# dusk-network/schnorr

Measured on NVIDIA B200. Metric: verifies_per_s, higher is better.
Workload: dtype u32

## Files before the change

schnorr_b200/csrc/constants_gen.cuh:

```cuda
#pragma once
#include <cstdint>
namespace sb200 {
#define SB200_FQ_MOD_INIT {0x00000001u, 0xffffffffu, 0xfffe5bfeu, 0x53bda402u, 0x09a1d805u, 0x3339d808u, 0x299d7d48u, 0x73eda753u}
#define SB200_FR_MOD_INIT {0xd6f72cb7u, 0xd0970e5eu, 0xccc81082u, 0xa6682093u, 0x01343b00u, 0x06673b01u, 0x6533afa9u, 0x0e7db4eau}
#define SB200_8R_INIT {0xb7b965b8u, 0x84b872f6u, 0x66408416u, 0x3341049eu, 0x09a1d805u, 0x3339d808u, 0x299d7d48u, 0x73eda753u}
#define SB200_FQ_ONE_INIT {0xfffffffeu, 0x00000001u, 0x00034802u, 0x5884b7fau, 0xecbc4ff5u, 0x998c4fefu, 0xacc5056fu, 0x1824b159u}
#define SB200_FQ_R2_INIT {0xf3f29c6du, 0xc999e990u, 0x87925c23u, 0x2b6cedcbu, 0x7254398fu, 0x05d31496u, 0x9f59ff11u, 0x0748d9d9u}
#define SB200_FR_R2_INIT {0x95e57731u, 0x67719aa4u, 0x9ce3fc26u, 0x51b0cef0u, 0xc026e9a5u, 0x69dab7fau, 0x8d127688u, 0x04f6547bu}
#define SB200_FR_NINV 0xef788ef9u
#define SB200_FQ_NINV 0xffffffffu
#define SB200_ED_D_INIT {0xb974f6b0u, 0x2a522455u, 0x0d9acab3u, 0xfc6cc9efu, 0xc27628d1u, 0x7a08fb94u, 0xfe0e262eu, 0x57f8f6a8u}
#define SB200_ED_2D_INIT {0x72e9ed5fu, 0x54a448acu, 0x1b373967u, 0xa51befdbu, 0x7b4a799eu, 0xc0d81f21u, 0xd27ecf14u, 0x3c0445feu}
#define SB200_G_U_INIT {0x547c71aau, 0xc8cd898cu, 0xb3564650u, 0x1e77bad0u, 0x49031ebeu, 0x0b5183a6u, 0xa3031a2cu, 0x4f54a483u}
#define SB200_G_V_INIT {0xffffffd9u, 0x00000026u, 0x003ffc27u, 0x3e1c038bu, 0x88581730u, 0x323016c6u, 0xa901ea00u, 0x56cb8254u}
#define SB200_GP_U_INIT {0x71c3e812u, 0x51d37e72u, 0x2074aaa8u, 0xf3ad4539u, 0xc0cfbca7u, 0x21bb2537u, 0x8bf29c9cu, 0x0bb82922u}
#define SB200_GP_V_INIT {0x0c68cf00u, 0x36fba2bfu, 0xd2b7f2adu, 0xcd442b52u, 0xf9f895d4u, 0xbe025c79u, 0x466dbd00u, 0x61e43e3fu}
#define SB200_FQ_ROOT_OF_UNITY_INIT {0x5f0e466au, 0xb9b58d8cu, 0x1819d7ecu, 0x5b1b4c80u, 0x52a31e64u, 0x0af53ae3u, 0x19e9b27bu, 0x5bf3addau}
#define SB200_FQ_SQRT_EXP_INIT {0x7fffffffu, 0x7fff2dffu, 0xa9ded201u, 0x04d0ec02u, 0x199cec04u, 0x94cebea4u, 0x39f6d3a9u, 0x00000000u}
#define SB200_FQ_SQRT_EXP_BITS 222
#define SB200_FQ_ISQRT_EXP_INIT {0x80000000u, 0x8000d1ffu, 0x561f89fdu, 0x4eecb800u, 0xf004ec01u, 0x9e6b1963u, 0xefa6a99eu, 0x73eda752u}
#define SB200_FQ_ISQRT_EXP_BITS 255
#define SB200_FQ_DLOG_W_INIT { \
  {0xfffffffeu, 0x00000001u, 0x00034802u, 0x5884b7fau, 0xecbc4ff5u, 0x998c4fefu, 0xacc5056fu, 0x1824b159u}, \
  {0x88202b65u, 0x1acf64e4u, 0x819f004fu, 0x5b18b637u, 0x3107fdf5u, 0xee649cabu, 0xce9012a0u, 0x27a8543du}, \
  {0x2c42eff8u, 0x6ecf4995u, 0x4d5dfa57u, 0x6ec1fa83u, 0x5656b15cu, 0x3ff5cf38u, 0x229e031bu, 0x54b80267u}, \
  {0x45c09c96u, 0x5fb40c77u, 0x8b8b1b1bu, 0xfff59b78u, 0x6b7eed47u, 0x023ba68bu, 0x76f3e130u, 0x4e17f66fu}, \
  {0xaa89cfb1u, 0xf3b05674u, 0x6006b9feu, 0x072f0140u, 0x25667a26u, 0xce9a0dbfu, 0x2d598374u, 0x4d2ce405u}, \
  {0x0b0a1289u, 0x25c2a002u, 0x7d082188u, 0x971c717fu, 0xd81ac5d8u, 0x4739dccau, 0xeee341c1u, 0x4f607ba9u}, \
  {0x3eb2a8ddu, 0x111f9842u, 0x6f38b840u, 0x1f772784u, 0x8e3ca13cu, 0xb28758a3u, 0xed9a48f0u, 0x5974f9f7u}, \
  {0xdcbeed53u, 0x0ddd2e46u, 0x33dbdd55u, 0xdf977d7fu, 0xc1470bbau, 0xdda3b36au, 0xb67a22b2u, 0x4818fbf6u}, \
  {0x00000003u, 0xfffffffdu, 0xfffb13fcu, 0xfb38ec08u, 0x1ce5880fu, 0x99ad8818u, 0x7cd877d8u, 0x5bc8f5f9u}, \
  {0x77dfd49cu, 0xe5309b1au, 0x7e5f5bafu, 0xf8a4edcbu, 0xd899da0fu, 0x44d53b5cu, 0x5b0d6aa7u, 0x4c455315u}, \
  {0xd3bd1009u, 0x9130b669u, 0xb2a061a7u, 0xe4fba97fu, 0xb34b26a8u, 0xf34408cfu, 0x06ff7a2cu, 0x1f35a4ecu}, \
  {0xba3f636bu, 0xa04bf387u, 0x747340e3u, 0x53c8088au, 0x9e22eabdu, 0x30fe317cu, 0xb2a99c18u, 0x25d5b0e3u}, \
  {0x55763050u, 0x0c4fa98au, 0x9ff7a200u, 0x4c8ea2c2u, 0xe43b5ddfu, 0x649fca48u, 0xfc43f9d3u, 0x26c0c34du}, \
  {0xf4f5ed78u, 0xda3d5ffcu, 0x82f63a76u, 0xbca13283u, 0x3187122cu, 0xebfffb3du, 0x3aba3b86u, 0x248d2ba9u}, \
  {0xc14d5724u, 0xeee067bcu, 0x90c5a3beu, 0x34467c7eu, 0x7b6536c9u, 0x80b27f64u, 0x3c033457u, 0x1a78ad5bu}, \
  {0x234112aeu, 0xf222d1b8u, 0xcc227ea9u, 0x74262683u, 0x485acc4au, 0x5596249du, 0x73235a95u, 0x2bd4ab5cu}, \
}
#define SB200_FQ_DLOG_P_INIT { \
  {0xfffffffeu, 0x00000001u, 0x00034802u, 0x5884b7fau, 0xecbc4ff5u, 0x998c4fefu, 0xacc5056fu, 0x1824b159u}, \
  {0xdcf3219au, 0x4256481au, 0x96b6cad3u, 0x45f37b7fu, 0x5f7a3b27u, 0xf9c3f1d7u, 0x658afd43u, 0x2d2fc049u}, \
  {0xb510e57eu, 0x1e4739c8u, 0x184b8322u, 0xcc6032ecu, 0x984f6527u, 0x67262f63u, 0x87e5e5d4u, 0x5f5b959au}, \
  {0x55ba3b5bu, 0x2c18ffe6u, 0xa301cb77u, 0x9f7c110du, 0x8987dc47u, 0xdc5921a2u, 0xb7e50ed6u, 0x2624052cu}, \
  {0x70de2c18u, 0x0491bcebu, 0x87989fc9u, 0xfe592990u, 0xb064bd3cu, 0x687fc87au, 0xfbd5ad87u, 0x184857c8u}, \
  {0x15d8086bu, 0x7da1ec25u, 0x0f895256u, 0xebefe178u, 0x6da44d28u, 0x7ccb4492u, 0x1418b341u, 0x0d341d07u}, \
  {0xa39260bdu, 0x371f6f57u, 0xb2adfd57u, 0x03233f13u, 0xe86e03e8u, 0xda6056f1u, 0x89616101u, 0x64e6ed21u}, \
  {0x5d68adabu, 0xc6213a40u, 0xf0bc64ebu, 0x717d6528u, 0x5a40ec6fu, 0x455a4aefu, 0x8c10c91du, 0x4b3801e3u}, \
  {0x54eb1d75u, 0x79675917u, 0xd07fc645u, 0x1d44be7du, 0x47873890u, 0x1fddcce9u, 0xd4a502f9u, 0x1c9bd17eu}, \
  {0xf41614dbu, 0x91d36fb2u, 0x2d5ee4f0u, 0xf0ca4660u, 0x97a3d0e0u, 0x358061cfu, 0x398358a9u, 0x1f710187u}, \
  {0x0e975eb0u, 0x573de590u, 0xfde6df69u, 0x45876f88u, 0x6fefa181u, 0x8ec11e78u, 0x47e325c6u, 0x3b82fc93u}, \
  {0x44c7342bu, 0x7d6cc6f9u, 0x9d3b75c2u, 0x5f804e66u, 0xfb977827u, 0xc787ac1bu, 0x242122d5u, 0x27cb0565u}, \
  {0x76ab126fu, 0xeda7545bu, 0x02493555u, 0xe69a0018u, 0xd36a1a77u, 0xbf43e82fu, 0x740a2463u, 0x66d7e2d2u}, \
  {0x287def7au, 0x25e3cfcbu, 0xf520ad2eu, 0x33e06f94u, 0xb53a8083u, 0x441ae296u, 0x9ac05dc5u, 0x4e335a86u}, \
  {0xd961433fu, 0x8b753cbdu, 0xb5ef3ca5u, 0x5510c621u, 0xdbe2dc3du, 0x1aed0940u, 0xbf547affu, 0x41202b7au}, \
  {0xd9f2b2e9u, 0x9ad76de6u, 0x69662643u, 0x767ed606u, 0x510ae26bu, 0x6f9e9b13u, 0x6b4afe61u, 0x6aea05a3u}, \
  {0xfffffffeu, 0x00000001u, 0x00034802u, 0x5884b7fau, 0xecbc4ff5u, 0x998c4fefu, 0xacc5056fu, 0x1824b159u}, \
  {0x7b483997u, 0x25909fe2u, 0x3f40368fu, 0xe6c3383bu, 0xdfbf158fu, 0xe7a72791u, 0x90ca2226u, 0x2bccc288u}, \
  {0x61b4a6dfu, 0x3bbb6d5fu, 0xb34eca42u, 0x029e0c54u, 0x3ffd89d1u, 0x1d4e3056u, 0xd07ec38bu, 0x6b3cb83cu}, \
  {0x2fe00938u, 0x6c0ecbb6u, 0xb0e2f081u, 0x464ce985u, 0x63e9f431u, 0x281f3d36u, 0x3c63c33du, 0x151b140du}, \
  {0x27c562bbu, 0xf6d82dbfu, 0x2b57637fu, 0x4ddc7290u, 0x06eab0a9u, 0xc17c34cdu, 0x2b59d621u, 0x068dfbaeu}, \
  {0x7f332db5u, 0x550dd9d7u, 0x50500ad0u, 0x7fc2c5eau, 0xa154e5f1u, 0x68b6c255u, 0x5175c276u, 0x6a14b04au}, \
  {0x3d579818u, 0xeac47c6du, 0xbd12a148u, 0x04cdb7a3u, 0x99cc35bau, 0xc74160d9u, 0x7ded3fd6u, 0x31552226u}, \
  {0x45feca49u, 0x07022427u, 0xe4b9af79u, 0x67ae65c8u, 0x33cd2d6bu, 0xd2aa9542u, 0x766209d0u, 0x4b7f6e39u}, \
  {0xae32dcdeu, 0xbd56d684u, 0x1409bd44u, 0x2db07b79u, 0x76a3e44eu, 0xf6fc95fcu, 0x24ed7b31u, 0x5adc0a48u}, \
  {0x9b8ac597u, 0x18faac24u, 0xad6a2e5eu, 0x03c5535eu, 0x1aeaa4c7u, 0x9516a609u, 0x0e93a59du, 0x4cf2c66fu}, \
  {0xb053e34bu, 0x22b855f1u, 0xa6a58337u, 0x99d367e2u, 0x6a6fed50u, 0x1a1b8fc9u, 0xaf1243eeu, 0x02be6719u}, \
  {0x56a1b05au, 0x4c899974u, 0x52a00333u, 0x92077279u, 0x3fb3e264u, 0x5b69a565u, 0xfd04f965u, 0x22894c17u}, \
  {0x76d4f9a2u, 0xaab13750u, 0x27b6e4cdu, 0x6e15f748u, 0xaad66ed8u, 0x5934218eu, 0x8b7fc61eu, 0x2d8fee11u}, \
  {0x22ba096cu, 0xda0e363bu, 0xe108034au, 0x73e94e78u, 0x03175cb2u, 0x16662707u, 0xdc289c5cu, 0x0935b070u}, \
  {0xba91d935u, 0x8710449fu, 0x10ba6380u, 0x74297a3cu, 0x3ed48ec8u, 0x1944fd71u, 0x230d1a6fu, 0x253baa10u}, \
  {0x45af1cb2u, 0x9912839cu, 0x0eff7d88u, 0x94ce8b8fu, 0x45d2192fu, 0x3d960b14u, 0xa970bf7eu, 0x0ab3e280u}, \
  {0xfffffffeu, 0x00000001u, 0x00034802u, 0x5884b7fau, 0xecbc4ff5u, 0x998c4fefu, 0xacc5056fu, 0x1824b159u}, \
  {0x990adacau, 0xad970bf0u, 0x35d536acu, 0xfcc75b77u, 0x776dcbaeu, 0x8dce37c6u, 0x0b26861du, 0x39f39d66u}, \
  {0x3f3f7413u, 0x62a17c8au, 0xbb17edbau, 0xf60c53c0u, 0x0c4e2817u, 0x4a9ea2d0u, 0xf7c560f3u, 0x13b632eeu}, \
  {0xbf8d2010u, 0xaa23c71fu, 0x1803ba5bu, 0x82408b4cu, 0xb0e69d63u, 0xe205f14cu, 0xc89b398eu, 0x35817d11u}, \
  {0xf6421a00u, 0x52c40fb8u, 0x5ec95569u, 0xbf33428eu, 0x0f71a346u, 0x5ecc78ddu, 0x9336bf44u, 0x5bb66cdbu}, \
  {0xd7a69137u, 0x9d39ae58u, 0xc8b94ac3u, 0x31aa9c79u, 0x01df0186u, 0x165f9fecu, 0xd00f8128u, 0x37fcf0ecu}, \
  {0x8830c83bu, 0xc5ad52beu, 0x3e94bc59u, 0x335c2573u, 0xf405e823u, 0x3e0d24a9u, 0xc983967du, 0x340c1cd8u}, \
  {0x5015e046u, 0xe0e15508u, 0x07f09bf5u, 0x89a013dbu, 0x756f0918u, 0x6a372ae3u, 0xa1a1661eu, 0x3f38e644u}, \
  {0xe3c30b08u, 0x9aa2ba63u, 0xd67b21bcu, 0xc3a07402u, 0x29af6349u, 0x64a4e583u, 0xf6ae051cu, 0x64bffb89u}, \
  {0x97e8c141u, 0x5c0656e3u, 0xde2270f4u, 0x9d2b3e00u, 0x0724a33au, 0x639a4ba0u, 0x8342d321u, 0x081ccecbu}, \
  {0x5eb65c76u, 0x2eb03e83u, 0x7c9d4f12u, 0x01c1e452u, 0x48471ba3u, 0x53c1e14fu, 0x46fa1afdu, 0x57191969u}, \
  {0x40374953u, 0x2176d8ceu, 0x348adbefu, 0xd5f2b8e9u, 0x0192e4aeu, 0x009ddad0u, 0x139e2bedu, 0x062b6996u}, \
  {0xc54c7224u, 0xa473141bu, 0x677c3a87u, 0xe5cc4b84u, 0xd657177cu, 0xc43f284bu, 0x13ede9e1u, 0x68f92b69u}, \
  {0x61e3b145u, 0xace2b2b2u, 0xb79bac80u, 0xe6ee1368u, 0x39d8c96bu, 0xcbc23989u, 0x7bdc8336u, 0x1679bcf7u}, \
  {0x19606f59u, 0x5e54cc69u, 0x72106cf8u, 0x9cc664a2u, 0xa8f39d52u, 0x7ac51b8au, 0xda01f7b5u, 0x6f6436c3u}, \
  {0xc1ce4a7au, 0xf0f3c50bu, 0x1b61b4a3u, 0xd3b7deadu, 0x360f0e9fu, 0x91827a03u, 0x6c77c17au, 0x6ac60dd2u}, \
  {0xfffffffeu, 0x00000001u, 0x00034802u, 0x5884b7fau, 0xecbc4ff5u, 0x998c4fefu, 0xacc5056fu, 0x1824b159u}, \
  {0xb64957f6u, 0x68ee7cb8u, 0x0a2b8bafu, 0x8eeda81eu, 0x256c4becu, 0xd749ce3du, 0x2ae8d689u, 0x48230b86u}, \
// ... 211 lines not shown
```

schnorr_b200/csrc/fq.cuh:

```cuda
#pragma once
#include <cstdint>

#include "constants_gen.cuh"

#if defined(__CUDACC__)
#define SB_HD __host__ __device__ __forceinline__
#define SB_D __device__ __forceinline__
#else
#define SB_HD inline
#define SB_D inline
#endif

namespace sb200 {

#ifndef SB_Q1_SHORTCUT
#define SB_Q1_SHORTCUT 0
#endif

struct fq {
  uint32_t v[8];
};

#if !defined(__CUDA_ARCH__)
namespace emu {
// ... 56 lines not shown
      "madc.lo.cc.u32 %6, %9, %13, %6;\n\t"
      "madc.hi.cc.u32 %7, %9, %13, %7;\n\t"
      "addc.u32 %8, %8, 0;"
      : "+r"(x[0]), "+r"(x[1]), "+r"(x[2]), "+r"(x[3]), "+r"(x[4]), "+r"(x[5]), "+r"(x[6]), "+r"(x[7]), "+r"(ytop)
      : "r"(a), "r"(b0), "r"(b2), "r"(b4), "r"(b6));
#else
  SB_COUNT(wide, 4);
  uint32_t c = emu::add_at(x, 8, 0, (uint64_t)a * b0, 0);
  c += emu::add_at(x, 8, 2, (uint64_t)a * b2, 0);
  c += emu::add_at(x, 8, 4, (uint64_t)a * b4, 0);
  c += emu::add_at(x, 8, 6, (uint64_t)a * b6, 0);
  ytop += c;
#endif
}

SB_HD void blk_mac_odd(uint32_t* y, uint32_t a, uint32_t b1, uint32_t b3, uint32_t b5, uint32_t b7) {
#if defined(__CUDA_ARCH__)
  asm("mad.lo.cc.u32 %0, %8, %9, %0;\n\t"
      "madc.hi.cc.u32 %1, %8, %9, %1;\n\t"
      "madc.lo.cc.u32 %2, %8, %10, %2;\n\t"
      "madc.hi.cc.u32 %3, %8, %10, %3;\n\t"
      "madc.lo.cc.u32 %4, %8, %11, %4;\n\t"
      "madc.hi.cc.u32 %5, %8, %11, %5;\n\t"
      "madc.lo.cc.u32 %6, %8, %12, %6;\n\t"
      "madc.hi.u32 %7, %8, %12, %7;"
      : "+r"(y[0]), "+r"(y[1]), "+r"(y[2]), "+r"(y[3]), "+r"(y[4]), "+r"(y[5]), "+r"(y[6]), "+r"(y[7])
      : "r"(a), "r"(b1), "r"(b3), "r"(b5), "r"(b7));
#else
  SB_COUNT(wide, 4);
  uint32_t c = emu::add_at(y, 8, 0, (uint64_t)a * b1, 0);
  c += emu::add_at(y, 8, 2, (uint64_t)a * b3, 0);
  c += emu::add_at(y, 8, 4, (uint64_t)a * b5, 0);
  c += emu::add_at(y, 8, 6, (uint64_t)a * b7, 0);
  (void)c;
#endif
}

SB_HD void blk_red_even_q(uint32_t* x, uint32_t& ytop, uint32_t m, uint32_t q2, uint32_t q4, uint32_t q6) {
#if defined(__CUDA_ARCH__)
  asm("mad.lo.cc.u32 %0, %7, %8, %0;\n\t"
      "madc.hi.cc.u32 %1, %7, %8, %1;\n\t"
      "madc.lo.cc.u32 %2, %7, %9, %2;\n\t"
      "madc.hi.cc.u32 %3, %7, %9, %3;\n\t"
      "madc.lo.cc.u32 %4, %7, %10, %4;\n\t"
      "madc.hi.cc.u32 %5, %7, %10, %5;\n\t"
      "addc.u32 %6, %6, 0;"
      : "+r"(x[2]), "+r"(x[3]), "+r"(x[4]), "+r"(x[5]), "+r"(x[6]), "+r"(x[7]), "+r"(ytop)
      : "r"(m), "r"(q2), "r"(q4), "r"(q6));
#else
  SB_COUNT(wide, 3);
  uint32_t c = emu::add_at(x, 8, 2, (uint64_t)m * q2, 0);
  c += emu::add_at(x, 8, 4, (uint64_t)m * q4, 0);
  c += emu::add_at(x, 8, 6, (uint64_t)m * q6, 0);
  ytop += c;
#endif
}

SB_HD void blk_red_odd_q(uint32_t* y, uint32_t m, uint32_t t0, uint32_t q3, uint32_t q5, uint32_t q7) {
#if defined(__CUDA_ARCH__)
  asm("{\n\t.reg .u32 h;\n\t"
      "min.u32 h, %8, 1;\n\t"
      "sub.u32 h, %8, h;\n\t"
      "add.cc.u32 %0, %0, %9;\n\t"
      "addc.cc.u32 %1, %1, h;\n\t"
      "madc.lo.cc.u32 %2, %8, %10, %2;\n\t"
      "madc.hi.cc.u32 %3, %8, %10, %3;\n\t"
      "madc.lo.cc.u32 %4, %8, %11, %4;\n\t"
      "madc.hi.cc.u32 %5, %8, %11, %5;\n\t"
      "madc.lo.cc.u32 %6, %8, %12, %6;\n\t"
      "madc.hi.u32 %7, %8, %12, %7;\n\t}"
      : "+r"(y[0]), "+r"(y[1]), "+r"(y[2]), "+r"(y[3]), "+r"(y[4]), "+r"(y[5]), "+r"(y[6]), "+r"(y[7])
      : "r"(m), "r"(t0), "r"(q3), "r"(q5), "r"(q7));
#else
  SB_COUNT(wide, 3);
  uint32_t hi1 = m - (m != 0 ? 1u : 0u);
  uint32_t c = emu::add_at(y, 8, 0, ((uint64_t)hi1 << 32) | t0, 0);
  c += emu::add_at(y, 8, 2, (uint64_t)m * q3, 0);
  c += emu::add_at(y, 8, 4, (uint64_t)m * q5, 0);
  c += emu::add_at(y, 8, 6, (uint64_t)m * q7, 0);
  (void)c;
#endif
}

SB_HD void blk_mac1c(uint32_t* acc, uint32_t a, uint32_t b0) {
#if defined(__CUDA_ARCH__)
  asm("mad.lo.cc.u32 %0, %3, %4, %0;\n\t"
      "madc.hi.cc.u32 %1, %3, %4, %1;\n\t"
      "addc.u32 %2, %2, 0;"
      : "+r"(acc[0]), "+r"(acc[1]), "+r"(acc[2])
      : "r"(a), "r"(b0));
#else
  SB_COUNT(wide, 1);
  acc[2] += emu::add_at(acc, 2, 0, (uint64_t)a * b0, 0);
#endif
}
SB_HD void blk_mac2c(uint32_t* acc, uint32_t a, uint32_t b0, uint32_t b1) {
#if defined(__CUDA_ARCH__)
  asm("mad.lo.cc.u32 %0, %5, %6, %0;\n\t"
      "madc.hi.cc.u32 %1, %5, %6, %1;\n\t"
      "madc.lo.cc.u32 %2, %5, %7, %2;\n\t"
      "madc.hi.cc.u32 %3, %5, %7, %3;\n\t"
      "addc.u32 %4, %4, 0;"
      : "+r"(acc[0]), "+r"(acc[1]), "+r"(acc[2]), "+r"(acc[3]), "+r"(acc[4])
      : "r"(a), "r"(b0), "r"(b1));
#else
  SB_COUNT(wide, 2);
  uint32_t c = emu::add_at(acc, 4, 0, (uint64_t)a * b0, 0);
  c += emu::add_at(acc, 4, 2, (uint64_t)a * b1, 0);
  acc[4] += c;
#endif
}
SB_HD void blk_mac3c(uint32_t* acc, uint32_t a, uint32_t b0, uint32_t b1, uint32_t b2) {
#if defined(__CUDA_ARCH__)
  asm("mad.lo.cc.u32 %0, %7, %8, %0;\n\t"
      "madc.hi.cc.u32 %1, %7, %8, %1;\n\t"
      "madc.lo.cc.u32 %2, %7, %9, %2;\n\t"
      "madc.hi.cc.u32 %3, %7, %9, %3;\n\t"
      "madc.lo.cc.u32 %4, %7, %10, %4;\n\t"
      "madc.hi.cc.u32 %5, %7, %10, %5;\n\t"
      "addc.u32 %6, %6, 0;"
      : "+r"(acc[0]), "+r"(acc[1]), "+r"(acc[2]), "+r"(acc[3]), "+r"(acc[4]), "+r"(acc[5]), "+r"(acc[6])
      : "r"(a), "r"(b0), "r"(b1), "r"(b2));
#else
  SB_COUNT(wide, 3);
  uint32_t c = emu::add_at(acc, 6, 0, (uint64_t)a * b0, 0);
  c += emu::add_at(acc, 6, 2, (uint64_t)a * b1, 0);
  c += emu::add_at(acc, 6, 4, (uint64_t)a * b2, 0);
  acc[6] += c;
#endif
}
SB_HD void blk_mac4c(uint32_t* acc, uint32_t a, uint32_t b0, uint32_t b1, uint32_t b2, uint32_t b3) {
  blk_mac_even(acc, acc[8], a, b0, b1, b2, b3);
}

SB_HD void blk_sqr_diag(uint32_t* t, const uint32_t* a) {
#if defined(__CUDA_ARCH__)
  asm("mad.lo.cc.u32 %0, %16, %16, %0;\n\t"
      "madc.hi.cc.u32 %1, %16, %16, %1;\n\t"
      "madc.lo.cc.u32 %2, %17, %17, %2;\n\t"
      "madc.hi.cc.u32 %3, %17, %17, %3;\n\t"
      "madc.lo.cc.u32 %4, %18, %18, %4;\n\t"
      "madc.hi.cc.u32 %5, %18, %18, %5;\n\t"
      "madc.lo.cc.u32 %6, %19, %19, %6;\n\t"
      "madc.hi.cc.u32 %7, %19, %19, %7;\n\t"
      "madc.lo.cc.u32 %8, %20, %20, %8;\n\t"
      "madc.hi.cc.u32 %9, %20, %20, %9;\n\t"
      "madc.lo.cc.u32 %10, %21, %21, %10;\n\t"
      "madc.hi.cc.u32 %11, %21, %21, %11;\n\t"
      "madc.lo.cc.u32 %12, %22, %22, %12;\n\t"
      "madc.hi.cc.u32 %13, %22, %22, %13;\n\t"
      "madc.lo.cc.u32 %14, %23, %23, %14;\n\t"
      "madc.hi.u32 %15, %23, %23, %15;"
      : "+r"(t[0]), "+r"(t[1]), "+r"(t[2]), "+r"(t[3]), "+r"(t[4]), "+r"(t[5]), "+r"(t[6]), "+r"(t[7]), "+r"(t[8]),
        "+r"(t[9]), "+r"(t[10]), "+r"(t[11]), "+r"(t[12]), "+r"(t[13]), "+r"(t[14]), "+r"(t[15])
      : "r"(a[0]), "r"(a[1]), "r"(a[2]), "r"(a[3]), "r"(a[4]), "r"(a[5]), "r"(a[6]), "r"(a[7]));
#else
  SB_COUNT(wide, 8);
  uint32_t c = 0;
  for (int i = 0; i < 8; i++) c += emu::add_at(t, 16, 2 * i, (uint64_t)a[i] * a[i], 0);
  (void)c;
#endif
}

SB_HD void merge_eo16(uint32_t* r, const uint32_t* e, const uint32_t* o) {
#if defined(__CUDA_ARCH__)
  r[0] = e[0];
  asm("add.cc.u32 %0, %15, %30;\n\t"
      "addc.cc.u32 %1, %16, %31;\n\t"
      "addc.cc.u32 %2, %17, %32;\n\t"
      "addc.cc.u32 %3, %18, %33;\n\t"
      "addc.cc.u32 %4, %19, %34;\n\t"
      "addc.cc.u32 %5, %20, %35;\n\t"
      "addc.cc.u32 %6, %21, %36;\n\t"
      "addc.cc.u32 %7, %22, %37;\n\t"
      "addc.cc.u32 %8, %23, %38;\n\t"
      "addc.cc.u32 %9, %24, %39;\n\t"
      "addc.cc.u32 %10, %25, %40;\n\t"
      "addc.cc.u32 %11, %26, %41;\n\t"
      "addc.cc.u32 %12, %27, %42;\n\t"
      "addc.cc.u32 %13, %28, %43;\n\t"
      "addc.u32 %14, %29, %44;"
      : "=r"(r[1]), "=r"(r[2]), "=r"(r[3]), "=r"(r[4]), "=r"(r[5]), "=r"(r[6]), "=r"(r[7]), "=r"(r[8]), "=r"(r[9]),
        "=r"(r[10]), "=r"(r[11]), "=r"(r[12]), "=r"(r[13]), "=r"(r[14]), "=r"(r[15])
      : "r"(e[1]), "r"(e[2]), "r"(e[3]), "r"(e[4]), "r"(e[5]), "r"(e[6]), "r"(e[7]), "r"(e[8]), "r"(e[9]), "r"(e[10]),
        "r"(e[11]), "r"(e[12]), "r"(e[13]), "r"(e[14]), "r"(e[15]), "r"(o[0]), "r"(o[1]), "r"(o[2]), "r"(o[3]), "r"(o[4]),
        "r"(o[5]), "r"(o[6]), "r"(o[7]), "r"(o[8]), "r"(o[9]), "r"(o[10]), "r"(o[11]), "r"(o[12]), "r"(o[13]), "r"(o[14]));
#else
  r[0] = e[0];
  uint64_t c = 0;
  for (int i = 1; i < 16; i++) {
    c += (uint64_t)e[i] + o[i - 1];
    r[i] = (uint32_t)c;
    c >>= 32;
  }
#endif
}

SB_HD uint32_t blk_fold_red_odd(uint32_t& x0, uint32_t xf, uint32_t tprev, uint32_t* y, uint32_t q1, uint32_t q3,
                                uint32_t q5, uint32_t q7) {
  uint32_t m;
#if defined(__CUDA_ARCH__)
  asm("{\n\t.reg .u32 t, h;\n\t"
      "add.cc.u32 t, %11, 0xffffffff;\n\t"
      "addc.cc.u32 %0, %0, %10;\n\t"
      "xor.b32 %9, %0, %12;\n\t"
      "add.u32 %9, %9, 1;\n\t"
      "min.u32 h, %9, 1;\n\t"
      "sub.u32 h, %9, h;\n\t"
      "addc.cc.u32 %1, %1, %0;\n\t"
      "addc.cc.u32 %2, %2, h;\n\t"
      "madc.lo.cc.u32 %3, %9, %13, %3;\n\t"
      "madc.hi.cc.u32 %4, %9, %13, %4;\n\t"
      "madc.lo.cc.u32 %5, %9, %14, %5;\n\t"
      "madc.hi.cc.u32 %6, %9, %14, %6;\n\t"
      "madc.lo.cc.u32 %7, %9, %15, %7;\n\t"
      "madc.hi.u32 %8, %9, %15, %8;\n\t}"
      : "+r"(x0), "+r"(y[0]), "+r"(y[1]), "+r"(y[2]), "+r"(y[3]), "+r"(y[4]), "+r"(y[5]), "+r"(y[6]), "+r"(y[7]), "=&r"(m)
      : "r"(xf), "r"(tprev), "r"(q1), "r"(q3), "r"(q5), "r"(q7));
#else
  SB_COUNT(wide, 4);
  uint64_t t = (uint64_t)x0 + xf + (tprev != 0 ? 1u : 0u);
  x0 = (uint32_t)t;
  uint32_t c = (uint32_t)(t >> 32);
  m = 0u - x0;
  SB_COUNT(wide, -1);
  (void)q1;
  c = emu::add_at(y, 8, 0, ((uint64_t)(m - (m != 0 ? 1u : 0u)) << 32) | x0, c);
  c += emu::add_at(y, 8, 2, (uint64_t)m * q3, 0);
  c += emu::add_at(y, 8, 4, (uint64_t)m * q5, 0);
  c += emu::add_at(y, 8, 6, (uint64_t)m * q7, 0);
  (void)c;
#endif
  return m;
}

SB_HD uint32_t add8(uint32_t* r, const uint32_t* a, const uint32_t* b) {
  uint32_t c;
#if defined(__CUDA_ARCH__)
  asm("add.cc.u32 %0, %9, %17;\n\t"
      "addc.cc.u32 %1, %10, %18;\n\t"
      "addc.cc.u32 %2, %11, %19;\n\t"
      "addc.cc.u32 %3, %12, %20;\n\t"
      "addc.cc.u32 %4, %13, %21;\n\t"
// ... 204 lines not shown
  mul_wide16(T, a.v, b.v);
  return mont_reduce16(T);
#endif
  uint32_t X[8], Y[8], xf = 0, tprev = 0;
#pragma unroll
  for (int i = 0; i < 8; i++) X[i] = Y[i] = 0;
  const uint32_t q1 = SB_FQ_MOD(1), q2 = SB_FQ_MOD(2), q3 = SB_FQ_MOD(3), q4 = SB_FQ_MOD(4), q5 = SB_FQ_MOD(5),
                 q6 = SB_FQ_MOD(6), q7 = SB_FQ_MOD(7);
#pragma unroll
  for (int i = 0; i < 8; i++) {
    uint32_t ai = a.v[i];
    blk_fold_mac_odd(X[0], xf, tprev, Y, ai, b.v[1], b.v[3], b.v[5], b.v[7]);
    blk_mac_even(X, Y[7], ai, b.v[0], b.v[2], b.v[4], b.v[6]);
    tprev = X[0];
#if defined(__CUDA_ARCH__) && SB_FQ_MOD_IMM
    uint32_t m;
    asm("xor.b32 %0, %1, %2;\n\tadd.u32 %0, %0, 1;" : "=r"(m) : "r"(tprev), "r"(q1));
#else
    uint32_t m = (tprev ^ q1) + 1u;
#endif
    blk_red_even_q(X, Y[7], m, q2, q4, q6);
#if SB_Q1_SHORTCUT
    blk_red_odd_q(Y, m, tprev, q3, q5, q7);
#else
    blk_mac_odd(Y, m, q1, q3, q5, q7);
#endif
    xf = X[1];
    uint32_t nx[8], ny[8];
#pragma unroll
    for (int k = 0; k < 8; k++) nx[k] = Y[k];
#pragma unroll
    for (int k = 0; k < 6; k++) ny[k] = X[k + 2];
    ny[6] = 0;
    ny[7] = 0;
#pragma unroll
    for (int k = 0; k < 8; k++) {
      X[k] = nx[k];
      Y[k] = ny[k];
    }
  }
  fq r;
  uint32_t s[8] = {xf, Y[0], Y[1], Y[2], Y[3], Y[4], Y[5], Y[6]};
  add8c(r.v, X, s, tprev);
  cond_sub_p<FqP>(r.v);
  return r;
}

SB_HD fq mont_reduce16(const uint32_t* t) {
  uint32_t X[8], Y[8], xf = 0, tprev = 0;
#pragma unroll
  for (int i = 0; i < 8; i++) {
    X[i] = t[i];
    Y[i] = 0;
  }
  const uint32_t q1 = SB_FQ_MOD(1), q2 = SB_FQ_MOD(2), q3 = SB_FQ_MOD(3), q4 = SB_FQ_MOD(4), q5 = SB_FQ_MOD(5),
                 q6 = SB_FQ_MOD(6), q7 = SB_FQ_MOD(7);
#pragma unroll
  for (int i = 0; i < 8; i++) {
    uint32_t m = blk_fold_red_odd(X[0], xf, tprev, Y, q1, q3, q5, q7);
    tprev = X[0];
    blk_red_even_q(X, Y[7], m, q2, q4, q6);
    xf = X[1];
    uint32_t nx[8], ny[8];
#pragma unroll
    for (int k = 0; k < 8; k++) nx[k] = Y[k];
#pragma unroll
    for (int k = 0; k < 6; k++) ny[k] = X[k + 2];
    ny[6] = 0;
    ny[7] = 0;
#pragma unroll
    for (int k = 0; k < 8; k++) {
      X[k] = nx[k];
      Y[k] = ny[k];
    }
  }
  fq v, r;
  uint32_t s[8] = {xf, Y[0], Y[1], Y[2], Y[3], Y[4], Y[5], Y[6]};
  add8c(v.v, X, s, tprev);
  add8(r.v, v.v, t + 8);
  cond_sub_p<FqP>(r.v);
  return r;
}

SB_HD fq fq_sqr_inl(const fq& x) {
  SB_COUNT(fq_sqr, 1);
  const uint32_t* a = x.v;
  uint32_t E[16], O[16];
#pragma unroll
  for (int i = 0; i < 16; i++) E[i] = O[i] = 0;
  blk_mac4c(O + 0, a[0], a[1], a[3], a[5], a[7]);
  blk_mac3c(E + 2, a[0], a[2], a[4], a[6]);
  blk_mac3c(O + 2, a[1], a[2], a[4], a[6]);
  blk_mac3c(E + 4, a[1], a[3], a[5], a[7]);
  blk_mac3c(O + 4, a[2], a[3], a[5], a[7]);
  blk_mac2c(E + 6, a[2], a[4], a[6]);
  blk_mac2c(O + 6, a[3], a[4], a[6]);
  blk_mac2c(E + 8, a[3], a[5], a[7]);
  blk_mac2c(O + 8, a[4], a[5], a[7]);
  blk_mac1c(E + 10, a[4], a[6]);
  blk_mac1c(O + 10, a[5], a[6]);
  blk_mac1c(E + 12, a[5], a[7]);
  blk_mac1c(O + 12, a[6], a[7]);
  uint32_t S[16], T[16];
  merge_eo16(S, E, O);
  T[0] = S[0] << 1;
#pragma unroll
  for (int i = 1; i < 16; i++) T[i] = (S[i] << 1) | (S[i - 1] >> 31);
  blk_sqr_diag(T, a);
  return mont_reduce16(T);
}

SB_HD void mul_wide16(uint32_t* T, const uint32_t* a, const uint32_t* b) {
  uint32_t E[18], O[18];
#pragma unroll
  for (int i = 0; i < 18; i++) E[i] = O[i] = 0;
#pragma unroll
  for (int i = 0; i < 8; i++) {
    if ((i & 1) == 0) {
      blk_mac4c(E + i, a[i], b[0], b[2], b[4], b[6]);
      blk_mac4c(O + i, a[i], b[1], b[3], b[5], b[7]);
    } else {
      blk_mac4c(O + i - 1, a[i], b[0], b[2], b[4], b[6]);
      blk_mac4c(E + i + 1, a[i], b[1], b[3], b[5], b[7]);
    }
  }
  merge_eo16(T, E, O);
}

SB_HD void acc17(uint32_t* S, const uint32_t* T) {
#if defined(__CUDA_ARCH__)
  asm("add.cc.u32 %0, %0, %17;\n\t"
      "addc.cc.u32 %1, %1, %18;\n\t"
      "addc.cc.u32 %2, %2, %19;\n\t"
      "addc.cc.u32 %3, %3, %20;\n\t"
      "addc.cc.u32 %4, %4, %21;\n\t"
      "addc.cc.u32 %5, %5, %22;\n\t"
      "addc.cc.u32 %6, %6, %23;\n\t"
      "addc.cc.u32 %7, %7, %24;\n\t"
      "addc.cc.u32 %8, %8, %25;\n\t"
      "addc.cc.u32 %9, %9, %26;\n\t"
      "addc.cc.u32 %10, %10, %27;\n\t"
      "addc.cc.u32 %11, %11, %28;\n\t"
      "addc.cc.u32 %12, %12, %29;\n\t"
      "addc.cc.u32 %13, %13, %30;\n\t"
      "addc.cc.u32 %14, %14, %31;\n\t"
      "addc.cc.u32 %15, %15, %32;\n\t"
      "addc.u32 %16, %16, 0;"
      : "+r"(S[0]), "+r"(S[1]), "+r"(S[2]), "+r"(S[3]), "+r"(S[4]), "+r"(S[5]), "+r"(S[6]), "+r"(S[7]), "+r"(S[8]),
        "+r"(S[9]), "+r"(S[10]), "+r"(S[11]), "+r"(S[12]), "+r"(S[13]), "+r"(S[14]), "+r"(S[15]), "+r"(S[16])
      : "r"(T[0]), "r"(T[1]), "r"(T[2]), "r"(T[3]), "r"(T[4]), "r"(T[5]), "r"(T[6]), "r"(T[7]), "r"(T[8]), "r"(T[9]),
        "r"(T[10]), "r"(T[11]), "r"(T[12]), "r"(T[13]), "r"(T[14]), "r"(T[15]));
#else
  uint64_t c = 0;
  for (int i = 0; i < 16; i++) {
    c += (uint64_t)S[i] + T[i];
    S[i] = (uint32_t)c;
    c >>= 32;
  }
  S[16] += (uint32_t)c;
#endif
}

SB_HD fq mont_reduce17(const uint32_t* S) {
  uint32_t X[8], Y[8], xf = 0, tprev = 0;
#pragma unroll
  for (int i = 0; i < 8; i++) {
    X[i] = S[i];
    Y[i] = 0;
  }
  const uint32_t q1 = SB_FQ_MOD(1), q2 = SB_FQ_MOD(2), q3 = SB_FQ_MOD(3), q4 = SB_FQ_MOD(4), q5 = SB_FQ_MOD(5),
                 q6 = SB_FQ_MOD(6), q7 = SB_FQ_MOD(7);
#pragma unroll
  for (int i = 0; i < 8; i++) {
    uint32_t m = blk_fold_red_odd(X[0], xf, tprev, Y, q1, q3, q5, q7);
    tprev = X[0];
    blk_red_even_q(X, Y[7], m, q2, q4, q6);
    xf = X[1];
    uint32_t nx[8], ny[8];
#pragma unroll
    for (int k = 0; k < 8; k++) nx[k] = Y[k];
#pragma unroll
    for (int k = 0; k < 6; k++) ny[k] = X[k + 2];
    ny[6] = 0;
    ny[7] = 0;
#pragma unroll
    for (int k = 0; k < 8; k++) {
      X[k] = nx[k];
      Y[k] = ny[k];
    }
  }
  fq v, r;
  uint32_t s[8] = {xf, Y[0], Y[1], Y[2], Y[3], Y[4], Y[5], Y[6]};
// ... 258 lines not shown
```

Measured before the change: 28.82 million.

## Interleave Fq squaring with Montgomery reduction row by row

Replaces the separate schoolbook squaring (even/odd accumulators, merge, doubling shift, diagonal add, then full 16-word Montgomery reduce) with a fused, row-interleaved squaring-plus-reduction. It uses pre-doubled operand words and a precomputed correction constant table. The aim is to remove the merge/shift passes and the separate reduction, which lowers instruction count and register pressure in the hot fq_sqr. The risk is correctness subtlety from the carry handling and the constant offsets.

```diff
diff --git a/schnorr_b200/csrc/constants_gen.cuh b/schnorr_b200/csrc/constants_gen.cuh
--- a/schnorr_b200/csrc/constants_gen.cuh
+++ b/schnorr_b200/csrc/constants_gen.cuh
@@ -6,6 +6,7 @@
 #define SB200_8R_INIT {0xb7b965b8u, 0x84b872f6u, 0x66408416u, 0x3341049eu, 0x09a1d805u, 0x3339d808u, 0x299d7d48u, 0x73eda753u}
 #define SB200_FQ_ONE_INIT {0xfffffffeu, 0x00000001u, 0x00034802u, 0x5884b7fau, 0xecbc4ff5u, 0x998c4fefu, 0xacc5056fu, 0x1824b159u}
 #define SB200_FQ_R2_INIT {0xf3f29c6du, 0xc999e990u, 0x87925c23u, 0x2b6cedcbu, 0x7254398fu, 0x05d31496u, 0x9f59ff11u, 0x0748d9d9u}
+#define SB200_FQ_SQR_K_INIT {0x00000000u, 0x00000000u, 0x00000000u, 0x00000000u, 0x00000000u, 0x00000000u, 0x00000000u, 0x65851279u, 0x5ec0f297u, 0x6fef090cu, 0x86629e98u, 0x7cd7c3e4u, 0x11442cd1u, 0x5c0c89afu, 0x9112bc50u, 0x00000000u}
 #define SB200_FR_R2_INIT {0x95e57731u, 0x67719aa4u, 0x9ce3fc26u, 0x51b0cef0u, 0xc026e9a5u, 0x69dab7fau, 0x8d127688u, 0x04f6547bu}
 #define SB200_FR_NINV 0xef788ef9u
 #define SB200_FQ_NINV 0xffffffffu
diff --git a/schnorr_b200/csrc/fq.cuh b/schnorr_b200/csrc/fq.cuh
--- a/schnorr_b200/csrc/fq.cuh
+++ b/schnorr_b200/csrc/fq.cuh
@@ -162,35 +162,35 @@
 #endif
 }
 
-SB_HD void blk_mac1c(uint32_t* acc, uint32_t a, uint32_t b0) {
+SB_HD void blk_mac1c(uint32_t* acc, uint32_t& top, uint32_t a, uint32_t b0) {
 #if defined(__CUDA_ARCH__)
   asm("mad.lo.cc.u32 %0, %3, %4, %0;\n\t"
       "madc.hi.cc.u32 %1, %3, %4, %1;\n\t"
       "addc.u32 %2, %2, 0;"
-      : "+r"(acc[0]), "+r"(acc[1]), "+r"(acc[2])
+      : "+r"(acc[0]), "+r"(acc[1]), "+r"(top)
       : "r"(a), "r"(b0));
 #else
   SB_COUNT(wide, 1);
-  acc[2] += emu::add_at(acc, 2, 0, (uint64_t)a * b0, 0);
-#endif
-}
-SB_HD void blk_mac2c(uint32_t* acc, uint32_t a, uint32_t b0, uint32_t b1) {
+  top += emu::add_at(acc, 2, 0, (uint64_t)a * b0, 0);
+#endif
+}
+SB_HD void blk_mac2c(uint32_t* acc, uint32_t& top, uint32_t a, uint32_t b0, uint32_t b1) {
 #if defined(__CUDA_ARCH__)
   asm("mad.lo.cc.u32 %0, %5, %6, %0;\n\t"
       "madc.hi.cc.u32 %1, %5, %6, %1;\n\t"
       "madc.lo.cc.u32 %2, %5, %7, %2;\n\t"
       "madc.hi.cc.u32 %3, %5, %7, %3;\n\t"
       "addc.u32 %4, %4, 0;"
-      : "+r"(acc[0]), "+r"(acc[1]), "+r"(acc[2]), "+r"(acc[3]), "+r"(acc[4])
+      : "+r"(acc[0]), "+r"(acc[1]), "+r"(acc[2]), "+r"(acc[3]), "+r"(top)
       : "r"(a), "r"(b0), "r"(b1));
 #else
   SB_COUNT(wide, 2);
   uint32_t c = emu::add_at(acc, 4, 0, (uint64_t)a * b0, 0);
   c += emu::add_at(acc, 4, 2, (uint64_t)a * b1, 0);
-  acc[4] += c;
-#endif
-}
-SB_HD void blk_mac3c(uint32_t* acc, uint32_t a, uint32_t b0, uint32_t b1, uint32_t b2) {
+  top += c;
+#endif
+}
+SB_HD void blk_mac3c(uint32_t* acc, uint32_t& top, uint32_t a, uint32_t b0, uint32_t b1, uint32_t b2) {
 #if defined(__CUDA_ARCH__)
   asm("mad.lo.cc.u32 %0, %7, %8, %0;\n\t"
       "madc.hi.cc.u32 %1, %7, %8, %1;\n\t"
@@ -199,46 +199,68 @@
       "madc.lo.cc.u32 %4, %7, %10, %4;\n\t"
       "madc.hi.cc.u32 %5, %7, %10, %5;\n\t"
       "addc.u32 %6, %6, 0;"
-      : "+r"(acc[0]), "+r"(acc[1]), "+r"(acc[2]), "+r"(acc[3]), "+r"(acc[4]), "+r"(acc[5]), "+r"(acc[6])
+      : "+r"(acc[0]), "+r"(acc[1]), "+r"(acc[2]), "+r"(acc[3]), "+r"(acc[4]), "+r"(acc[5]), "+r"(top)
       : "r"(a), "r"(b0), "r"(b1), "r"(b2));
 #else
   SB_COUNT(wide, 3);
   uint32_t c = emu::add_at(acc, 6, 0, (uint64_t)a * b0, 0);
   c += emu::add_at(acc, 6, 2, (uint64_t)a * b1, 0);
   c += emu::add_at(acc, 6, 4, (uint64_t)a * b2, 0);
-  acc[6] += c;
+  top += c;
 #endif
 }
 SB_HD void blk_mac4c(uint32_t* acc, uint32_t a, uint32_t b0, uint32_t b1, uint32_t b2, uint32_t b3) {
   blk_mac_even(acc, acc[8], a, b0, b1, b2, b3);
 }
 
-SB_HD void blk_sqr_diag(uint32_t* t, const uint32_t* a) {
-#if defined(__CUDA_ARCH__)
-  asm("mad.lo.cc.u32 %0, %16, %16, %0;\n\t"
-      "madc.hi.cc.u32 %1, %16, %16, %1;\n\t"
-      "madc.lo.cc.u32 %2, %17, %17, %2;\n\t"
-      "madc.hi.cc.u32 %3, %17, %17, %3;\n\t"
-      "madc.lo.cc.u32 %4, %18, %18, %4;\n\t"
-      "madc.hi.cc.u32 %5, %18, %18, %5;\n\t"
-      "madc.lo.cc.u32 %6, %19, %19, %6;\n\t"
-      "madc.hi.cc.u32 %7, %19, %19, %7;\n\t"
-      "madc.lo.cc.u32 %8, %20, %20, %8;\n\t"
-      "madc.hi.cc.u32 %9, %20, %20, %9;\n\t"
-      "madc.lo.cc.u32 %10, %21, %21, %10;\n\t"
-      "madc.hi.cc.u32 %11, %21, %21, %11;\n\t"
-      "madc.lo.cc.u32 %12, %22, %22, %12;\n\t"
-      "madc.hi.cc.u32 %13, %22, %22, %13;\n\t"
-      "madc.lo.cc.u32 %14, %23, %23, %14;\n\t"
-      "madc.hi.u32 %15, %23, %23, %15;"
-      : "+r"(t[0]), "+r"(t[1]), "+r"(t[2]), "+r"(t[3]), "+r"(t[4]), "+r"(t[5]), "+r"(t[6]), "+r"(t[7]), "+r"(t[8]),
-        "+r"(t[9]), "+r"(t[10]), "+r"(t[11]), "+r"(t[12]), "+r"(t[13]), "+r"(t[14]), "+r"(t[15])
-      : "r"(a[0]), "r"(a[1]), "r"(a[2]), "r"(a[3]), "r"(a[4]), "r"(a[5]), "r"(a[6]), "r"(a[7]));
-#else
-  SB_COUNT(wide, 8);
-  uint32_t c = 0;
-  for (int i = 0; i < 8; i++) c += emu::add_at(t, 16, 2 * i, (uint64_t)a[i] * a[i], 0);
-  (void)c;
+SB_HD void blk_mac1(uint32_t* acc, uint32_t a, uint32_t b0) {
+#if defined(__CUDA_ARCH__)
+  asm("mad.lo.cc.u32 %0, %2, %3, %0;\n\t"
+      "madc.hi.u32 %1, %2, %3, %1;"
+      : "+r"(acc[0]), "+r"(acc[1])
+      : "r"(a), "r"(b0));
+#else
+  SB_COUNT(wide, 1);
+  emu::add_at(acc, 2, 0, (uint64_t)a * b0, 0);
+#endif
+}
+
+SB_HD void blk_sqr_red_row(uint32_t* x, uint32_t* y, uint32_t xf, uint32_t q1, uint32_t q2p, uint32_t q3, uint32_t q4,
+                           uint32_t q5, uint32_t q6, uint32_t q7) {
+#if defined(__CUDA_ARCH__)
+  asm("{\n\t.reg .u32 m;\n\t"
+      "add.cc.u32 %0, %0, %14;\n\t"
+      "xor.b32 m, %0, %15;\n\t"
+      "addc.cc.u32 %1, %1, %0;\n\t"
+      "madc.lo.cc.u32 %2, m, %16, %2;\n\t"
+      "madc.hi.cc.u32 %3, m, %16, %3;\n\t"
+      "madc.lo.cc.u32 %4, m, %18, %4;\n\t"
+      "madc.hi.cc.u32 %5, m, %18, %5;\n\t"
+      "madc.lo.cc.u32 %6, m, %20, %6;\n\t"
+      "madc.hi.cc.u32 %7, m, %20, %7;\n\t"
+      "addc.u32 %13, %13, 0;\n\t"
+      "mad.lo.cc.u32 %8, m, %17, %8;\n\t"
+      "madc.hi.cc.u32 %9, m, %17, %9;\n\t"
+      "madc.lo.cc.u32 %10, m, %19, %10;\n\t"
+      "madc.hi.cc.u32 %11, m, %19, %11;\n\t"
+      "madc.lo.cc.u32 %12, m, %21, %12;\n\t"
+      "madc.hi.u32 %13, m, %21, %13;\n\t}"
+      : "+r"(x[0]), "+r"(x[1]), "+r"(x[2]), "+r"(x[3]), "+r"(x[4]), "+r"(x[5]), "+r"(x[6]), "+r"(x[7]), "+r"(y[2]),
+        "+r"(y[3]), "+r"(y[4]), "+r"(y[5]), "+r"(y[6]), "+r"(y[7])
+      : "r"(xf), "r"(q1), "r"(q2p), "r"(q3), "r"(q4), "r"(q5), "r"(q6), "r"(q7));
+#else
+  SB_COUNT(wide, 6);
+  uint64_t t = (uint64_t)x[0] + xf;
+  x[0] = (uint32_t)t;
+  const uint32_t m = x[0] ^ q1;
+  uint32_t c = emu::add_at(x, 8, 1, x[0], (uint32_t)(t >> 32));
+  c += emu::add_at(x, 8, 2, (uint64_t)m * q2p, 0);
+  c += emu::add_at(x, 8, 4, (uint64_t)m * q4, 0);
+  c += emu::add_at(x, 8, 6, (uint64_t)m * q6, 0);
+  y[7] += c;
+  emu::add_at(y, 8, 2, (uint64_t)m * q3, 0);
+  emu::add_at(y, 8, 4, (uint64_t)m * q5, 0);
+  emu::add_at(y, 8, 6, (uint64_t)m * q7, 0);
 #endif
 }
 
@@ -609,32 +631,69 @@
   return r;
 }
 
+SB_HD void sqr_row(uint32_t* X, uint32_t* Y, const uint32_t* a, const uint32_t* d, int r) {
+  uint32_t b[8];
+#pragma unroll
+  for (int j = 0; j < 8; j++) b[j] = j == r ? a[r] : j == r + 1 ? a[j] << 1 : d[j];
+  const uint32_t ar = a[r];
+  switch ((r | 1) / 2) {
+    case 0: blk_mac_even(X, Y[7], ar, b[1], b[3], b[5], b[7]); break;
+    case 1: blk_mac3c(X + 2, Y[7], ar, b[3], b[5], b[7]); break;
+    case 2: blk_mac2c(X + 4, Y[7], ar, b[5], b[7]); break;
+    default: blk_mac1c(X + 6, Y[7], ar, b[7]); break;
+  }
+  switch ((r + 1) / 2) {
+    case 0:
+    case 1: blk_mac3c(Y, Y[6], ar, b[2], b[4], b[6]); break;
+    case 2: blk_mac2c(Y + 2, Y[6], ar, b[4], b[6]); break;
+    default: blk_mac1c(Y + 4, Y[6], ar, b[6]); break;
+  }
+}
+
 SB_HD fq fq_sqr_inl(const fq& x) {
   SB_COUNT(fq_sqr, 1);
   const uint32_t* a = x.v;
-  uint32_t E[16], O[16];
-#pragma unroll
-  for (int i = 0; i < 16; i++) E[i] = O[i] = 0;
-  blk_mac4c(O + 0, a[0], a[1], a[3], a[5], a[7]);
-  blk_mac3c(E + 2, a[0], a[2], a[4], a[6]);
-  blk_mac3c(O + 2, a[1], a[2], a[4], a[6]);
-  blk_mac3c(E + 4, a[1], a[3], a[5], a[7]);
-  blk_mac3c(O + 4, a[2], a[3], a[5], a[7]);
-  blk_mac2c(E + 6, a[2], a[4], a[6]);
-  blk_mac2c(O + 6, a[3], a[4], a[6]);
-  blk_mac2c(E + 8, a[3], a[5], a[7]);
-  blk_mac2c(O + 8, a[4], a[5], a[7]);
-  blk_mac1c(E + 10, a[4], a[6]);
-  blk_mac1c(O + 10, a[5], a[6]);
-  blk_mac1c(E + 12, a[5], a[7]);
-  blk_mac1c(O + 12, a[6], a[7]);
-  uint32_t S[16], T[16];
-  merge_eo16(S, E, O);
-  T[0] = S[0] << 1;
-#pragma unroll
-  for (int i = 1; i < 16; i++) T[i] = (S[i] << 1) | (S[i - 1] >> 31);
-  blk_sqr_diag(T, a);
-  return mont_reduce16(T);
+  const uint32_t k[16] = SB200_FQ_SQR_K_INIT;
+  uint32_t d[8], X[8], Y[8], xf = 0;
+  d[0] = 0;
+#pragma unroll
+  for (int j = 1; j < 8; j++) {
+#if defined(__CUDA_ARCH__)
+    d[j] = __funnelshift_l(a[j - 1], a[j], 1);
+#else
+    d[j] = (a[j] << 1) | (a[j - 1] >> 31);
+#endif
+  }
+#pragma unroll
+  for (int i = 0; i < 8; i++) X[i] = Y[i] = 0;
+  Y[6] = k[7];
+  const uint32_t q1 = SB_FQ_MOD(1), q2p = FqP::p(2) + 1u, q3 = SB_FQ_MOD(3), q4 = SB_FQ_MOD(4), q5 = SB_FQ_MOD(5),
+                 q6 = SB_FQ_MOD(6), q7 = SB_FQ_MOD(7);
+  blk_mac1(X, a[0], a[0]);
+#pragma unroll
+  for (int i = 0; i < 8; i++) {
+    if (i > 0) sqr_row(X, Y, a, d, i - 1);
+    blk_sqr_red_row(X, Y, xf, q1, q2p, q3, q4, q5, q6, q7);
+    xf = X[1];
+    uint32_t nx[8], ny[8];
+#pragma unroll
+    for (int j = 0; j < 8; j++) nx[j] = Y[j];
+#pragma unroll
+    for (int j = 0; j < 6; j++) ny[j] = X[j + 2];
+    ny[6] = k[i + 8];
+    ny[7] = 0;
+#pragma unroll
+    for (int j = 0; j < 8; j++) {
+      X[j] = nx[j];
+      Y[j] = ny[j];
+    }
+  }
+  blk_mac1(X + 6, a[7], a[7]);
+  fq r;
+  const uint32_t s[8] = {xf, Y[0], Y[1], Y[2], Y[3], Y[4], Y[5], Y[6]};
+  add8(r.v, X, s);
+  cond_sub_p<FqP>(r.v);
+  return r;
 }
 
 SB_HD void mul_wide16(uint32_t* T, const uint32_t* a, const uint32_t* b) {
```

Measured after the change: 30.10 million, median of 6. 4.5% higher.
